# zakuro-ai/asr

Hardware: AMD Instinct MI355X
Metric: utterances/sec (10 s, 161-bin) DS2 5x1024 BiGRU CTC train step (higher is better)
Workload: dtype bf16

## Files before the change

### asr_amd/_lib.py

```python
from __future__ import annotations

import ctypes as C
import os
from typing import Optional

_HERE = os.path.dirname(os.path.abspath(__file__))
LIB_PATH = os.environ.get("DS2_LIB_PATH") or os.path.join(_HERE, "lib", "libds2hip.so")

_lib: Optional[C.CDLL] = None

vp, i32, i64, f32, f64, sz = C.c_void_p, C.c_int, C.c_longlong, C.c_float, C.c_double, C.c_size_t

SIGNATURES = {
    "ds2_version": (C.c_char_p, []),
    "ds2_last_error": (C.c_char_p, []),
    "ds2_device_info": (i32, [C.POINTER(i32), C.POINTER(i32), C.c_char_p, i32]),
    "ds2_debug_flags": (i32, [vp, i32]),
    "ds2_rnn_ctx_init": (i32, [vp, vp, vp, vp]),
    "ds2_memset_async": (i32, [vp, i32, sz, vp]),
    "ds2_ablation_build": (i32, []),
    "ds2_rnn_persistent_status": (i32, [vp, vp]),
    "ds2_rnn_persistent_counters": (i32, [vp, vp]),
    "ds2_rnn_poison_if_starved": (i32, [vp, vp, sz, vp]),
    "ds2_rnn_poison_seen": (i32, [vp]),
    "ds2_rnn_step_gate": (i32, [vp, vp, vp, vp]),
    "ds2_rnn_persistent_enable": (i32, [vp, i32, i32]),
    "ds2_rnn_last_path": (i32, [vp]),
    "ds2_rnn_bwd_ksplit_footprint": (i32, [i32, i32, C.POINTER(i32)]),
    "ds2_gemm_f32_workspace_bytes": (sz, [i32, i32, i32, i32]),
    "ds2_gemm_f32": (i32, [i32, i32, i32, i32, i32, vp, i32, i64, vp, i32, i64, vp, i32, i64, vp, i32, i32, i32, vp, sz, vp]),
    "ds2_gemm_bf16_workspace_bytes": (sz, [i32, i32, i32, i32]),
    "ds2_conv1_fwd_bf16_stat_blocks": (i32, [i32, i32, i32]),
    "ds2_conv1_fwd_bf16_stats": (i32, [vp, vp, vp, vp, vp, i32, i32, i32, vp, vp]),
    "ds2_conv2_fwd_bf16_stat_blocks": (i32, [i32, i32, i32]),
    "ds2_conv2_fwd_bf16_stats": (i32, [vp, vp, vp, vp, vp, i32, i32, i32, vp, vp]),
    "ds2_chanstats_from_partials_workspace_bytes": (sz, []),
    "ds2_chanstats_from_partials": (i32, [vp, i32, i32, f64, vp, vp, vp, vp, f32, vp, sz, vp]),
    "ds2_gemm_bf16_tn": (i32, [i32, i32, i32, vp, i32, i64, vp, i32, i64, vp, i32, i64, i32, i32, i32, vp, sz, vp]),
    "ds2_gemm_bf16_tn_group": (i32, [i32, vp, i32, vp]),
    "ds2_gemm_bf16_tn_splitk_group_workspace_bytes": (sz, [i32, vp, i32]),
    "ds2_gemm_bf16_tn_splitk_group": (i32, [i32, vp, i32, vp, sz, vp]),
    "ds2_gemm_bf16_tn_splitk_group_ep": (i32, [i32, vp, i32, i32, vp, vp, vp, vp, sz, vp]),
    "ds2_gemm_bf16_nt": (i32, [i32, i32, i32, vp, i32, i64, vp, i32, i64, vp, i32, i64, vp, i32, i32, i32, vp, sz, vp]),
    "ds2_cast_bf16": (i32, [vp, i32, vp, i32, i32, i32, vp]),
    "ds2_gemm_bf16_nt_obf16": (i32, [i32, i32, i32, vp, i32, vp, i32, vp, i32, vp, vp]),
    "ds2_cast_f32_from_bf16": (i32, [vp, vp, i64, vp]),
    "ds2_rnn_fwd_x": (i32, [vp, i32, vp, vp, vp, vp, vp, vp, vp, i32, i32, i32, vp, vp, vp, vp, sz, vp]),
    "ds2_split_bf16": (i32, [vp, i32, vp, i32, i32, i32, i32, vp]),
    "ds2_cast_transpose_bf16": (i32, [vp, i32, vp, i32, i32, i32, vp]),
    "ds2_cast_bf16_both_workspace_bytes": (sz, [i32, i32]),
    "ds2_cast_bf16_both": (i32, [vp, i32, vp, i32, vp, i32, i32, i32, vp, vp, sz, vp]),
    "ds2_transpose_bf16": (i32, [vp, i32, vp, i32, i32, i32, vp, vp, sz, vp]),
    "ds2_colreduce_workspace_bytes": (sz, [i32, i32]),
    "ds2_colstats_f32": (i32, [vp, i32, i32, i32, vp, vp, vp, vp, f32, vp, sz, vp]),
    "ds2_add_colstats_f32": (i32, [vp, i32, vp, i32, vp, i32, i32, i32, vp, vp, vp, vp, f32, vp, sz, vp]),
    "ds2_colsum_f32": (i32, [vp, i32, i32, i32, vp, vp, vp, sz, vp]),
    "ds2_bn1d_apply_f32": (i32, [vp, i32, vp, i32, i32, i32, vp, vp, vp, vp, f32, vp]),
    "ds2_bn1d_apply_bf16": (i32, [vp, i32, vp, i32, i32, i32, vp, vp, vp, vp, f32, vp]),
    "ds2_bn1d_bwd_f32": (i32, [vp, i32, vp, i32, vp, i32, i32, i32, vp, vp, vp, f32, vp, vp, vp, sz, vp]),
    "ds2_bn1d_bwd_xbf16": (i32, [vp, i32, vp, i32, vp, i32, i32, i32, vp, vp, vp, f32, vp, vp, vp, sz, vp]),
    "ds2_center_colstats": (i32, [vp, i32, vp, i32, vp, i32, vp, i32, i32, i32, vp, vp, vp, vp, vp, f32, vp, sz, vp]),
    "ds2_wih_fold_bf16": (i32, [vp, i32, vp, i32, i32, vp, vp, vp, vp, f32, vp, i32, vp, vp, vp, vp]),
    "ds2_scale_rank1_f32": (i32, [vp, i32, i32, i32, vp, vp, vp, vp]),
    "ds2_chanreduce_workspace_bytes": (sz, [i32]),
    "ds2_bn2d_stats_f32": (i32, [vp, i32, i32, i32, i32, vp, vp, vp, vp, f32, vp, sz, vp]),
# ... 150 lines not shown
```

### asr_amd/csrc/gemm_bf16.hip

```cpp
#include "common.h"
#include <type_traits>
#include <cstdint>
#include <stdlib.h>
#include <string.h>

namespace {

typedef __bf16 bf16x8 __attribute__((ext_vector_type(8)));
typedef __bf16 bf16x4 __attribute__((ext_vector_type(4)));
typedef float f32x2 __attribute__((ext_vector_type(2)));

constexpr int BM = 128, BN = 128, BK = 64;
constexpr int TN_MAX_PROBLEMS = 16;
constexpr int PITCH = 144;
constexpr int TILE_BYTES = BM * PITCH;

__device__ __attribute__((aligned(16))) float g_zero16[4] = {0.f, 0.f, 0.f, 0.f};
__device__ __attribute__((aligned(16))) float g_sink16[4];

struct BArgs {
  const __bf16* A; const __bf16* B; float* C; const float* bias;
  int M, N, K, lda, ldb, ldc;
  long long sA, sB, sC;
  int splitk, kchunk, accumulate;
// ... 986 lines not shown
    p.to_slab = nslab > 1;
    p.slab0 = term * splitk;
    p.nslab = (term == 0 && nslab > 1) ? nslab : 0;
    if (term == 0) {
      p.partial = (float*)((char*)workspace + off);
      if (nslab > 1) { off += (size_t)nslab * q.M * q.N * sizeof(float); elems += (long long)q.M * q.N / 4; any_slab = true; }
    } else {
      p.partial = g.p[i - term].partial;
    }
  }
  for (int i = nprob; i < TN_MAX_PROBLEMS; ++i) { g.p[i] = g.p[0]; g.p[i].nslab = 0; }
  g.nprob = nprob; g.splitk = splitk; g.nitems = items;
  g.ep_prob = ep_index; g.ep_scale = ep_scale; g.ep_rowv = ep_rowv; g.ep_shift = ep_shift;
  if (ep_index >= 0 && g.p[ep_index].nslab == 0) return 1;
  if (any_slab) DS2_REQUIRE(workspace && workspace_bytes >= off, "ds2_gemm_bf16_tn_splitk_group: workspace too small");
  DS2_ATTR_ONCE((gemm_bf16_tn_glds_kernel<true>), G_LDS);
  bool w4 = ds2_is_gfx950();
  for (int i = 0; i < nprob; ++i) {
    const ds2_tn_problem& q = probs[i];
    const int kc = g.p[i].kchunk, klast = q.K - (splitk - 1) * kc;
    w4 = w4 && (q.K % 64) == 0 && kc >= 128 && klast >= 128 && (long long)q.lda * 128 < (1ll << 31) && (long long)q.ldb * 128 < (1ll << 31);
  }
  if (w4) {
    DS2_ATTR_ONCE(gemm_bf16_tn_w4_kernel, W4_LDS);
    hipLaunchKernelGGL(gemm_bf16_tn_w4_kernel, dim3(items), dim3(256), W4_LDS, (hipStream_t)stream, g);
    DS2_LAUNCH_CHECK("gemm_bf16_tn_w4_kernel");
  } else {
    BArgs unused{};
    hipLaunchKernelGGL(gemm_bf16_tn_glds_kernel<true>, dim3(items), dim3(512), G_LDS, (hipStream_t)stream, unused, 0, 0, g);
    DS2_LAUNCH_CHECK("gemm_bf16_tn_glds_kernel<grouped>");
  }
  if (any_slab) {
    int blocks = (int)((elems + 255) / 256);
    if (blocks > 8192) blocks = 8192;
    hipLaunchKernelGGL(splitk_reduce_group_kernel, dim3(blocks), dim3(256), 0, (hipStream_t)stream, g, elems);
    DS2_LAUNCH_CHECK("splitk_reduce_group_kernel");
  }
  return 0;
}

extern "C" int ds2_gemm_bf16_tn_group(int nprob, const ds2_tn_problem* probs, int max_workgroups, void* stream) {
  DS2_REQUIRE(nprob >= 1 && nprob <= TNG_MAX_PROBLEMS && probs, "ds2_gemm_bf16_tn_group: 1..%d problems", TNG_MAX_PROBLEMS);
  TnGroup g;
  int tiles = 0;
  for (int i = 0; i < nprob; ++i) {
    const ds2_tn_problem& q = probs[i];
    DS2_REQUIRE(q.A && q.B && q.C && q.M >= 8 && q.N >= 8 && q.K > 0, "ds2_gemm_bf16_tn_group: problem %d: bad dims M=%d N=%d K=%d", i, q.M, q.N, q.K);
    DS2_REQUIRE((q.M % 8) == 0 && (q.N % 8) == 0 && (q.lda % 8) == 0 && (q.ldb % 8) == 0 && q.lda >= q.M && q.ldb >= q.N && q.ldc >= q.N,
                "ds2_gemm_bf16_tn_group: problem %d: M, N, lda, ldb must be multiples of 8 (M=%d N=%d lda=%d ldb=%d)", i, q.M, q.N, q.lda, q.ldb);
    DS2_REQUIRE(((uintptr_t)q.A % 16) == 0 && ((uintptr_t)q.B % 16) == 0, "ds2_gemm_bf16_tn_group: problem %d: operands must be 16-byte aligned", i);
    TnProb& p = g.p[i];
    p.A = (const __bf16*)q.A; p.B = (const __bf16*)q.B; p.C = q.C;
    p.M = q.M; p.N = q.N; p.K = q.K; p.lda = q.lda; p.ldb = q.ldb; p.ldc = q.ldc;
    p.ntx = ceil_div(q.N, 128);
    p.first_tile = tiles;
    tiles += p.ntx * ceil_div(q.M, 128);
  }
  for (int i = nprob; i < TNG_MAX_PROBLEMS; ++i) g.p[i] = g.p[0];
  g.nprob = nprob; g.ntiles = tiles;
  const int cus = ds2_cus_current() < 8 ? 8 : ds2_cus_current();
  int grid = max_workgroups > 0 ? (max_workgroups < cus ? max_workgroups : cus) : cus;
// ... 132 lines not shown
```

### asr_amd/csrc/gemm_tn_w4.h

```cpp
__global__ __launch_bounds__(256) void gemm_bf16_tn_w4_kernel(TnSGroup grp) {
  extern __shared__ __attribute__((aligned(1024))) char ldsg[];
  const __bf16* A;
  const __bf16* B;
  int pM, pN, plda, pldb, zs, orig, nt, kchunk, ntx, pK;
  float* Cfinal; float* Cslab; long long ldcf;
  bool partial;
  {
    const int item = tn_item_order(grp.nitems);
    A = grp.p[0].A; B = grp.p[0].B; Cfinal = grp.p[0].C; Cslab = grp.p[0].partial;
    pM = grp.p[0].M; pN = grp.p[0].N; pK = grp.p[0].K; plda = grp.p[0].lda; pldb = grp.p[0].ldb; ldcf = grp.p[0].ldc; ntx = grp.p[0].ntx;
    nt = grp.p[0].ntiles; kchunk = grp.p[0].kchunk;
    int first = 0, slab0 = grp.p[0].slab0, to_slab = grp.p[0].to_slab;
#pragma unroll
    for (int k = 1; k < TN_MAX_PROBLEMS; ++k)
      if (k < grp.nprob && item >= grp.p[k].first_item) {
        A = grp.p[k].A; B = grp.p[k].B; Cfinal = grp.p[k].C; Cslab = grp.p[k].partial;
        pM = grp.p[k].M; pN = grp.p[k].N; pK = grp.p[k].K; plda = grp.p[k].lda; pldb = grp.p[k].ldb; ldcf = grp.p[k].ldc; ntx = grp.p[k].ntx;
        nt = grp.p[k].ntiles; kchunk = grp.p[k].kchunk; first = grp.p[k].first_item; slab0 = grp.p[k].slab0; to_slab = grp.p[k].to_slab;
      }
    const int local = item - first;
    zs = local / nt; orig = local % nt;
    partial = to_slab != 0;
    Cslab += (long long)(slab0 + zs) * pM * pN;
  }
  const int m0 = (orig / ntx) * 256, n0 = (orig % ntx) * 256;
  const int kbeg = zs * kchunk;
  const int kend = min(pK, kbeg + kchunk);
  const int nkt = (kend - kbeg) >> 6;
  const int lane = threadIdx.x & 63;
  const int wave = __builtin_amdgcn_readfirstlane(threadIdx.x >> 6);
  const int wm = wave >> 1, wn = wave & 1;
  const unsigned lds0 = (unsigned)(uintptr_t)(lds_void*)ldsg;

  unsigned voffA[8], voffB[8];
#pragma unroll
  for (int i = 0; i < 8; ++i) {
    const int r = (wave + 4 * i) * 2 + (lane >> 5);
    const int gs = (lane & 31) ^ (((r & 3) << 2) | (((r >> 3) & 1) << 1));
    voffA[i] = (unsigned)(r * plda * 2 + min(m0 + gs * 8, pM - 8) * 2);
    voffB[i] = (unsigned)(r * pldb * 2 + min(n0 + gs * 8, pN - 8) * 2);
  }
  const char* sA = reinterpret_cast<const char*>(A + (long long)kbeg * plda);
  const char* sB = reinterpret_cast<const char*>(B + (long long)kbeg * pldb);
  const long long stepA = (long long)plda * 128, stepB = (long long)pldb * 128;
  const unsigned dstw = lds0 + wave * 1024;
  auto dma_a = [&](unsigned boff, int p) { w4_dma(voffA[p], sA, dstw + boff + p * 4096); };
  auto dma_b = [&](unsigned boff, int p) { w4_dma(voffB[p], sB, dstw + boff + 32768 + p * 4096); };

  const int p16 = lane & 15, q4 = p16 >> 2, g4 = lane >> 4;
  const unsigned rowpart = (unsigned)((g4 * 8 + q4) * 512);
  const unsigned xv = (unsigned)((q4 << 2) | ((g4 & 1) << 1));
  unsigned va[8], vb[8];
#pragma unroll
  for (int i = 0; i < 8; ++i) {
    const int ca = wm * 128 + i * 16 + 4 * (p16 & 3), cb = wn * 128 + i * 16 + 4 * (p16 & 3);
    va[i] = lds0 + rowpart + ((((ca >> 3) ^ xv) << 4) | (((ca >> 2) & 1) << 3));
    vb[i] = lds0 + 32768 + rowpart + ((((cb >> 3) ^ xv) << 4) | (((cb >> 2) & 1) << 3));
  }

  f32x4 acc[8][8];
  f32x4 fa[2][8], fb[2][8];
#define TW_BC(x) __builtin_bit_cast(bf16x8, x)
#define TW_SB() __builtin_amdgcn_sched_barrier(0)
#define TW_RD(dst, addr, off)                                                                                                         \
  do {                                                                                                                                \
    f32x2 lo_, hi_;                                                                                                                   \
    asm volatile("ds_read_b64_tr_b16 %0, %2 offset:%3\n\tds_read_b64_tr_b16 %1, %2 offset:%4"                                         \
                 : "=&v"(lo_), "=&v"(hi_)                                                                                             \
                 : "v"(addr), "n"(off), "n"((off) + 2048));                                                                           \
    dst = __builtin_shufflevector(lo_, hi_, 0, 1, 2, 3);                                                                              \
  } while (0)
#define TW_LGKM0(F)                                                                                                                   \
  asm volatile("s_waitcnt lgkmcnt(0)"                                                                                                 \
               : "+v"(F[0]), "+v"(F[1]), "+v"(F[2]), "+v"(F[3]), "+v"(F[4]), "+v"(F[5]), "+v"(F[6]), "+v"(F[7])                       \
               :                                                                                                                      \
               : "memory")
#define TW_KTILE(DMA, VMW, NEXT)                                                                                                      \
  do {                                                                                                                                \
    TW_SB();                                                                                                                          \
    _Pragma("unroll") for (int m_ = 0; m_ < 64; ++m_) {                                                                               \
      acc[m_ & 7][m_ >> 3] = __builtin_amdgcn_mfma_f32_16x16x32_bf16(TW_BC(fb[0][m_ >> 3]), TW_BC(fa[0][m_ & 7]), acc[m_ & 7][m_ >> 3], 0, 0, 0); \
// ... 13 lines not shown
    _Pragma("unroll") for (int m_ = 0; m_ < 64; ++m_) {                                                                               \
      acc[m_ & 7][m_ >> 3] = __builtin_amdgcn_mfma_f32_16x16x32_bf16(TW_BC(fb[1][m_ >> 3]), TW_BC(fa[1][m_ & 7]), acc[m_ & 7][m_ >> 3], 0, 0, 0); \
      TW_SB();                                                                                                                        \
      if ((DMA) && m_ < 10 && !(m_ & 1)) dma_b(boff, 3 + (m_ >> 1));                                                                  \
      if ((DMA) && m_ == 9) { sA += stepA; sB += stepB; }                                                                             \
      if ((NEXT) && m_ == 10) asm volatile(VMW ::: "memory");                                                                         \
      if ((NEXT) && m_ == 11) __builtin_amdgcn_s_barrier();                                                                           \
      if (m_ >= 13 && m_ <= 58 && (m_ - 13) % 3 == 0) {                                                                               \
        if ((m_ - 13) / 3 < 8) {                                                                                                      \
          va[((m_ - 13) / 3) & 7] ^= 65536u;                                                                                          \
          if (NEXT) TW_RD(fa[0][((m_ - 13) / 3) & 7], va[((m_ - 13) / 3) & 7], 0);                                                    \
        } else {                                                                                                                      \
          vb[((m_ - 13) / 3 - 8) & 7] ^= 65536u;                                                                                      \
          if (NEXT) TW_RD(fb[0][((m_ - 13) / 3 - 8) & 7], vb[((m_ - 13) / 3 - 8) & 7], 0);                                            \
        }                                                                                                                             \
      }                                                                                                                               \
      TW_SB();                                                                                                                        \
    }                                                                                                                                 \
    if (NEXT) { TW_LGKM0(fa[0]); TW_LGKM0(fb[0]); }                                                                                   \
    TW_SB();                                                                                                                          \
    boff ^= 65536u;                                                                                                                   \
  } while (0)

#pragma unroll
  for (int p = 0; p < 8; ++p) { dma_a(0u, p); dma_b(0u, p); }
  sA += stepA; sB += stepB;
#pragma unroll
  for (int p = 0; p < 8; ++p) { dma_a(65536u, p); dma_b(65536u, p); }
  sA += stepA; sB += stepB;
#pragma unroll
  for (int i = 0; i < 8; ++i)
#pragma unroll
    for (int j = 0; j < 8; ++j) acc[i][j] = f32x4{0.f, 0.f, 0.f, 0.f};
  asm volatile("s_waitcnt vmcnt(0)" ::: "memory");
  __builtin_amdgcn_s_barrier();
  TW_SB();
#pragma unroll
  for (int i = 0; i < 8; ++i) TW_RD(fa[0][i], va[i], 0);
#pragma unroll
  for (int j = 0; j < 8; ++j) TW_RD(fb[0][j], vb[j], 0);
  TW_LGKM0(fa[0]);
  TW_LGKM0(fb[0]);
  unsigned boff = 0u;
  int kt = 0;
  if (nkt > 2) {
    TW_KTILE(1, "", 1);
    kt = 1;
  }
  for (; kt < nkt - 2; ++kt) TW_KTILE(1, "s_waitcnt vmcnt(16)", 1);
  if (kt < nkt - 1) TW_KTILE(0, "s_waitcnt vmcnt(0)", 1);
  TW_KTILE(0, "", 0);

  {
    float* C = partial ? Cslab : Cfinal;
    const long long ldc = partial ? (long long)pN : ldcf;
    int el = lane;
    asm volatile("" : "+v"(el));
    const int frow = el & 15, fseg = el >> 4;
#pragma unroll
    for (int i = 0; i < 8; ++i) {
      const int row = m0 + wm * 128 + i * 16 + frow;
#pragma unroll
      for (int j = 0; j < 8; ++j) {
        const int col = n0 + wn * 128 + j * 16 + fseg * 4;
        if (row < pM && col < pN) *reinterpret_cast<f32x4*>(C + (long long)row * ldc + col) = acc[i][j];
      }
    }
  }
#undef TW_BC
#undef TW_SB
#undef TW_RD
#undef TW_LGKM0
#undef TW_KTILE
}
```

### asr_amd/engine.py

```python
from __future__ import annotations

from dataclasses import dataclass, field
from typing import Dict, List, Optional

import torch

from . import _lib, ops

Tensor = torch.Tensor
import os as _os
def _tune(name: str, default: str) -> str:
    return _os.environ.get(name, default) if _os.environ.get("DS2_EXPERIMENTAL") == "1" else default


OVERLAP_MODE = _tune("DS2_OVERLAP", "2")
OVERLAP_WGRAD = OVERLAP_MODE == "1"
WGRAD_TN = _tune("DS2_WGRAD_TN", "1") != "0"
CONV_STATS = _tune("DS2_CONV_STATS", "1") != "0"
FUSE_BN_BWD = _tune("DS2_FUSE_BN_BWD", "1") != "0"
WGRAD_SIDE = _tune("DS2_WGRAD_SIDE", "sk")
WGRAD_IDLE = _tune("DS2_WGRAD_IDLE", "1") != "0"
WGRAD_IDLE_MIN_CUS = int(_tune("DS2_WGRAD_IDLE_MIN_CUS", "64"))
F32_GEMM = _os.environ.get("DS2_F32_GEMM", "split")


F32_RNN = _os.environ.get("DS2_F32_RNN", "split")


F32_CONV = _os.environ.get("DS2_F32_CONV", "split")
F32_CONV_FWD = _tune("DS2_F32_CONV_FWD", "f32")
CONV2_WGRAD = _tune("DS2_CONV2_WGRAD", "nhwc")
GX_BF16 = _tune("DS2_GX_BF16", "0") != "0"
WS_PREARM = _tune("DS2_WS_PREARM", "1") != "0"
BN_FOLD = _tune("DS2_BN_FOLD", "1") != "0"
BN_FOLD_IDLE = _tune("DS2_BN_FOLD_IDLE", "1") != "0"


def _f32_split_ok(M: int, N: int, K: int, H: int = 8) -> bool:
    return F32_GEMM == "split" and M >= 512 and N >= 256 and K >= 256 and K % 8 == 0 and N % 8 == 0 and H % 8 == 0


_BWD_PERSISTENT = {}
_SIDE = {}
# ... 324 lines not shown
        rows = 2 * H if G == 3 else G * H
        ra, rb = (slice(B, M), slice(0, M - B)), (slice(0, M - B), slice(B, M))
        ops.gemm_bf16_tn_pair(dgx_bf[ra[0], 0:rows], dgx_bf[ra[1], G * H:G * H + rows], h_bf[rb[0], 0:H], h_bf[rb[1], H:2 * H], dwhh[:, :rows])
        if G == 3:
            ops.gemm_bf16_tn_pair(dhn_bf[ra[0], 0:H], dhn_bf[ra[1], H:2 * H], h_bf[rb[0], 0:H], h_bf[rb[1], H:2 * H], dwhh[:, 2 * H:])
        dwih = Gr[f"rnns.{l}.wih_cat"]
        I = dwih.shape[1]
        if I % 8 == 0:
            ops.gemm_bf16_tn(dgx_bf, xn[:, :I], out=dwih)
        else:
            dwih.copy_(ops.gemm_bf16_tn(dgx_bf, xn)[:, :I])
        fold_epilogue(l)
        done(f"rnns.{l}")

    def weight_gradients_group(l, dgx_bf, dhn_bf, h_bf, xn, on_side, start):
        dwhh, dwih = Gr[f"rnns.{l}.whh_cat"], Gr[f"rnns.{l}.wih_cat"]
        rows = 2 * H if G == 3 else G * H
        probs = [(dgx_bf, xn[:, :dwih.shape[1]], dwih),
                 (dgx_bf[B:M, 0:rows], h_bf[0:M - B, 0:H], dwhh[0, :rows]),
                 (dgx_bf[0:M - B, G * H:G * H + rows], h_bf[B:M, H:2 * H], dwhh[1, :rows])]
        if G == 3:
            probs += [(dhn_bf[B:M, 0:H], h_bf[0:M - B, 0:H], dwhh[0, 2 * H:]), (dhn_bf[0:M - B, H:2 * H], h_bf[B:M, H:2 * H], dwhh[1, 2 * H:])]
        f = fold_of.get(l)
        if WGRAD_SIDE == "sk" and f:
            def launch(pr):
                ops.gemm_bf16_tn_splitk_group(pr, epilogue=(0, f[0], Gr[f"rnns.{l}.bih_cat"].view(-1), f[1]))
        elif WGRAD_SIDE == "sk":
            launch = ops.gemm_bf16_tn_splitk_group
        else:
            def launch(pr):
                ops.gemm_bf16_tn_group(pr)
                fold_epilogue(l)
        if not on_side:
            launch(probs)
            done(f"rnns.{l}")
            return
        with torch.cuda.stream(side):
            side.wait_event(start)
            launch(probs)
            if not serial_buckets:
                done(f"rnns.{l}")
        if serial_buckets:
            main.wait_stream(side)
            done(f"rnns.{l}")
        for t in (dgx_bf, dhn_bf, h_bf, xn):
            if t is not None:
                t.record_stream(side)
        ctx.side_used = True

    shape_key = (ops.rnn_ctx_key(dev), G, H, B)

# ... 347 lines not shown
```

### asr_amd/ops.py

```python
from __future__ import annotations

import ctypes as C
import math
import threading
from typing import Optional, Tuple

import torch

from . import _lib

Tensor = torch.Tensor
BN_EPS = 1e-5
BN_MOMENTUM = 0.1


def _ptr(t: Optional[Tensor]):
    return None if t is None else t.data_ptr()


def _stream():
    return torch.cuda.current_stream().cuda_stream


def _chk_f32(*ts):
# ... 358 lines not shown
                break
            rounds = -(-tiles * s_ // 256)
            util = tiles * s_ / (rounds * 256.0)
            cost = 2.0 * mn * kmin / (1.1e15 * util) + (0.0 if s_ == 1 else (s_ + 1) * mn * 4 / 3e12)
            if best_cost is None or cost < best_cost * 0.97:
                best, best_cost = s_, cost
        splitk = best
    ap = C.cast(arr, C.c_void_p)
    wsb = lib.ds2_gemm_bf16_tn_splitk_group_workspace_bytes(len(problems), ap, splitk)
    ws = _ws(wsb, problems[0][0].device) if wsb else None
    if epilogue is not None:
        idx, scale, rowv, shift = epilogue
        _chk_f32(scale, rowv, shift)
        rc = lib.ds2_gemm_bf16_tn_splitk_group_ep(len(problems), ap, splitk, int(idx), scale.data_ptr(), rowv.data_ptr(), shift.data_ptr(), _ptr(ws), wsb, _stream())
        if rc == 0:
            return splitk
        if rc != 1:
            _lib.check(rc, "ds2_gemm_bf16_tn_splitk_group_ep")
        _lib.check(lib.ds2_gemm_bf16_tn_splitk_group(len(problems), ap, splitk, _ptr(ws), wsb, _stream()), "ds2_gemm_bf16_tn_splitk_group")
        scale_rank1_(problems[idx][2], scale, rowv, shift)
        return splitk
    _lib.check(lib.ds2_gemm_bf16_tn_splitk_group(len(problems), ap, splitk, _ptr(ws), wsb, _stream()), "ds2_gemm_bf16_tn_splitk_group")
    return splitk


def gemm_bf16_tn_group(problems, max_workgroups: int = 0):
    lib = _lib.load()
    arr = (_lib.TnProblem * len(problems))()
    for q, (A, B, out) in zip(arr, problems):
        assert A.dtype == torch.bfloat16 and B.dtype == torch.bfloat16 and out.dtype == torch.float32 and A.is_cuda and B.is_cuda and out.is_cuda
        assert A.dim() == 2 and B.dim() == 2 and out.dim() == 2 and A.stride(1) == 1 and B.stride(1) == 1 and out.stride(1) == 1
        K, M = A.shape
        assert B.size(0) == K and tuple(out.shape) == (M, B.size(1)), (A.shape, B.shape, out.shape)
        q.A, q.B, q.C = A.data_ptr(), B.data_ptr(), out.data_ptr()
        q.M, q.N, q.K, q.lda, q.ldb, q.ldc = M, B.size(1), K, _row_pitch(A), _row_pitch(B), _row_pitch(out)
    _lib.check(lib.ds2_gemm_bf16_tn_group(len(problems), C.cast(arr, C.c_void_p), int(max_workgroups), _stream()), "ds2_gemm_bf16_tn_group")


def colstats(X: Tensor, run_mean: Optional[Tensor] = None, run_var: Optional[Tensor] = None):
    _chk_f32(X, run_mean, run_var)
    lib = _lib.load()
    M, H = X.shape
    mean = torch.empty(H, dtype=torch.float32, device=X.device)
    var = torch.empty_like(mean)
    wsb = lib.ds2_colreduce_workspace_bytes(M, H)
    ws = _ws(wsb, X.device)
# ... 1191 lines not shown
```

### include/ds2hip.h

```cpp
#ifndef DS2HIP_H
#define DS2HIP_H

#include <stddef.h>
#include <stdint.h>

#ifdef __cplusplus
extern "C" {
#endif

const char* ds2_version(void);
const char* ds2_last_error(void);
int ds2_device_info(int* cu_count, int* wave_size, char* arch, int arch_len);
int ds2_ablation_build(void);

typedef struct ds2_rnn_ctx {
  int size;
  int persist_fwd, persist_bwd;
  int cooldown;
  int rearm_calls;
  int starved_total;
  int last_path;
  int last_bwd_kind;
  int debug_flags;
  int ws_prearmed;
// ... 9 lines not shown
size_t ds2_gemm_f32_workspace_bytes(int M, int N, int batch, int splitk);
int ds2_gemm_f32(int transA, int transB, int M, int N, int K, const float* A, int lda, long long strideA, const float* B, int ldb,
                 long long strideB, float* C, int ldc, long long strideC, const float* bias, int accumulate, int batch, int splitk,
                 void* workspace, size_t workspace_bytes, void* stream);

size_t ds2_gemm_bf16_workspace_bytes(int M, int N, int batch, int splitk);
int ds2_gemm_bf16_nt(int M, int N, int K, const void* A, int lda, long long strideA, const void* B, int ldb, long long strideB, float* C,
                     int ldc, long long strideC, const float* bias, int accumulate, int batch, int splitk, void* workspace,
                     size_t workspace_bytes, void* stream);
int ds2_gemm_bf16_nt_obf16(int M, int N, int K, const void* A, int lda, const void* B, int ldb, void* C, int ldc, const float* bias, void* stream);
int ds2_cast_f32_from_bf16(const void* src, float* dst, long long n, void* stream);
int ds2_gemm_bf16_tn(int M, int N, int K, const void* A, int lda, long long strideA, const void* B, int ldb, long long strideB, float* C,
                     int ldc, long long strideC, int accumulate, int batch, int splitk, void* workspace, size_t workspace_bytes,
                     void* stream);
typedef struct ds2_tn_problem {
  const void* A; const void* B; float* C;
  int M, N, K, lda, ldb, ldc;
} ds2_tn_problem;
int ds2_gemm_bf16_tn_group(int nprob, const ds2_tn_problem* problems, int max_workgroups, void* stream);
size_t ds2_gemm_bf16_tn_splitk_group_workspace_bytes(int nprob, const ds2_tn_problem* problems, int splitk);
int ds2_gemm_bf16_tn_splitk_group(int nprob, const ds2_tn_problem* problems, int splitk, void* workspace, size_t workspace_bytes, void* stream);
int ds2_gemm_bf16_tn_splitk_group_ep(int nprob, const ds2_tn_problem* probs, int splitk, int ep_index, const float* ep_scale, const float* ep_rowv,
                                     const float* ep_shift, void* workspace, size_t workspace_bytes, void* stream);
int ds2_cast_bf16(const float* src, int ld_src, void* dst, int ld_dst, int R, int Cc, void* stream);
int ds2_split_bf16(const float* src, int ld_src, void* dst, int ld_dst, int R, int Cc, int order, void* stream);
int ds2_cast_transpose_bf16(const float* src, int ld_src, void* dst, int ld_dst, int R, int Cc, void* stream);
size_t ds2_cast_bf16_both_workspace_bytes(int R, int Cc);
int ds2_cast_bf16_both(const float* src, int ld_src, void* dst_r, int ld_r, void* dst_t, int ld_t, int R, int Cc, float* colsum, void* ws,
                       size_t ws_bytes, void* stream);
int ds2_transpose_bf16(const void* src, int ld_src, void* dst_t, int ld_t, int R, int Cc, float* colsum, void* ws, size_t ws_bytes,
                       void* stream);

size_t ds2_colreduce_workspace_bytes(int M, int H);
int ds2_colstats_f32(const float* X, int ldx, int M, int H, float* mean, float* var, float* run_mean, float* run_var, float momentum,
                     void* ws, size_t ws_bytes, void* stream);
int ds2_add_colstats_f32(const float* Xa, int lda, const float* Xb, int ldb, float* Y, int ldy, int M, int H, float* mean, float* var,
                         float* run_mean, float* run_var, float momentum, void* ws, size_t ws_bytes, void* stream);
int ds2_colsum_f32(const float* X, int ldx, int M, int H, float* sum, float* sumsq, void* ws, size_t ws_bytes, void* stream);
int ds2_bn1d_apply_f32(const float* X, int ldx, float* Y, int ldy, int M, int H, const float* mean, const float* var,
                       const float* gamma, const float* beta, float eps, void* stream);
int ds2_bn1d_apply_bf16(const float* X, int ldx, void* Y, int ldy, int M, int H, const float* mean, const float* var, const float* gamma,
                        const float* beta, float eps, void* stream);
int ds2_bn1d_bwd_f32(const float* dY, int lddy, const float* X, int ldx, float* dX, int lddx, int M, int H, const float* mean,
                     const float* var, const float* gamma, float eps, float* dgamma, float* dbeta, void* ws, size_t ws_bytes,
                     void* stream);

// ... 244 lines not shown
```

Before: 2803.

## Add stream-K style run-partitioned grouped TN wgrad GEMM with cached host plans

Adds a persistent 'runs' variant of the w4 grouped TN GEMM. A host-side planner cuts the total K-tile work across all problems into near-equal contiguous runs, one per workgroup sized to the CU count. Each workgroup loops over its segments and writes partial tiles to slabs, which are reduced afterwards. Plans and device tables are cached per shape. The aim is to remove load imbalance and tail waves from fixed split-K for the RNN weight-gradient GEMMs, at the cost of extra slab traffic and a reduction pass. It is enabled by default for non-side-stream launches and falls back to split-K when the shapes are ineligible.

```diff
diff --git a/asr_amd/_lib.py b/asr_amd/_lib.py
--- a/asr_amd/_lib.py
+++ b/asr_amd/_lib.py
@@ -41,6 +41,9 @@
     "ds2_gemm_bf16_tn_splitk_group_workspace_bytes": (sz, [i32, vp, i32]),
     "ds2_gemm_bf16_tn_splitk_group": (i32, [i32, vp, i32, vp, sz, vp]),
     "ds2_gemm_bf16_tn_splitk_group_ep": (i32, [i32, vp, i32, i32, vp, vp, vp, vp, sz, vp]),
+    "ds2_gemm_bf16_tn_runs_group_workspace_bytes": (sz, [i32, vp, i32]),
+    "ds2_gemm_bf16_tn_runs_group": (i32, [i32, vp, i32, vp, sz, vp]),
+    "ds2_gemm_bf16_tn_runs_group_ep": (i32, [i32, vp, i32, i32, vp, vp, vp, vp, sz, vp]),
     "ds2_gemm_bf16_nt": (i32, [i32, i32, i32, vp, i32, i64, vp, i32, i64, vp, i32, i64, vp, i32, i32, i32, vp, sz, vp]),
     "ds2_cast_bf16": (i32, [vp, i32, vp, i32, i32, i32, vp]),
     "ds2_gemm_bf16_nt_obf16": (i32, [i32, i32, i32, vp, i32, vp, i32, vp, i32, vp, vp]),
diff --git a/asr_amd/csrc/gemm_bf16.hip b/asr_amd/csrc/gemm_bf16.hip
--- a/asr_amd/csrc/gemm_bf16.hip
+++ b/asr_amd/csrc/gemm_bf16.hip
@@ -1,4 +1,7 @@
 #include "common.h"
+#include "tn_runs_plan.h"
+#include <map>
+#include <mutex>
 #include <type_traits>
 #include <cstdint>
 #include <stdlib.h>
@@ -1032,8 +1035,9 @@
     w4 = w4 && (q.K % 64) == 0 && kc >= 128 && klast >= 128 && (long long)q.lda * 128 < (1ll << 31) && (long long)q.ldb * 128 < (1ll << 31);
   }
   if (w4) {
-    DS2_ATTR_ONCE(gemm_bf16_tn_w4_kernel, W4_LDS);
-    hipLaunchKernelGGL(gemm_bf16_tn_w4_kernel, dim3(items), dim3(256), W4_LDS, (hipStream_t)stream, g);
+    DS2_ATTR_ONCE((gemm_bf16_tn_w4_kernel<false>), W4_LDS);
+    hipLaunchKernelGGL((gemm_bf16_tn_w4_kernel<false>), dim3(items), dim3(256), W4_LDS, (hipStream_t)stream, g, (const TnRunsSeg*)nullptr,
+                       (const int*)nullptr);
     DS2_LAUNCH_CHECK("gemm_bf16_tn_w4_kernel");
   } else {
     BArgs unused{};
@@ -1047,6 +1051,126 @@
     DS2_LAUNCH_CHECK("splitk_reduce_group_kernel");
   }
   return 0;
+}
+
+namespace {
+struct TnRunsCached {
+  TnRunsPlan plan;
+  void* table = nullptr;
+  size_t seg_off = 0;
+};
+std::mutex g_tn_runs_mutex;
+std::map<std::vector<int>, TnRunsCached>& tn_runs_cache() { static std::map<std::vector<int>, TnRunsCached> c; return c; }
+
+bool tn_runs_eligible(int nprob, const ds2_tn_problem* probs) {
+  if (nprob < 1 || nprob > TN_MAX_PROBLEMS || !probs || !ds2_is_gfx950()) return false;
+  for (int i = 0; i < nprob; ++i) {
+    const ds2_tn_problem& q = probs[i];
+    if (q.K < 128 || (q.K % 64) != 0 || q.M < 8 || q.N < 8) return false;
+    if ((long long)q.lda * 128 >= (1ll << 31) || (long long)q.ldb * 128 >= (1ll << 31)) return false;
+    if (i > 0 && probs[i - 1].C == q.C) return false;
+  }
+  return true;
+}
+TnRunsCached* tn_runs_lookup(int nprob, const ds2_tn_problem* probs, int max_workgroups, bool upload, void* stream) {
+  int gmax = ds2_cus_current();
+  if (max_workgroups > 0 && max_workgroups < gmax) gmax = max_workgroups;
+  std::vector<int> key{ds2_dev_index(), gmax, nprob};
+  int Ms[TN_MAX_PROBLEMS], Ns[TN_MAX_PROBLEMS], Ks[TN_MAX_PROBLEMS];
+  for (int i = 0; i < nprob; ++i) {
+    Ms[i] = probs[i].M; Ns[i] = probs[i].N; Ks[i] = probs[i].K;
+    key.push_back(Ms[i]); key.push_back(Ns[i]); key.push_back(Ks[i]);
+  }
+  const int G = tn_runs_pick_groups(tn_runs_tiles(nprob, Ms, Ns), gmax);
+  std::lock_guard<std::mutex> lock(g_tn_runs_mutex);
+  auto& cache = tn_runs_cache();
+  auto it = cache.find(key);
+  if (it == cache.end()) {
+    if (cache.size() >= 256) return nullptr;
+    TnRunsCached c;
+    if (!tn_runs_plan(nprob, Ms, Ns, Ks, G, &c.plan)) return nullptr;
+    if (!c.plan.nphase && G != gmax && !tn_runs_plan(nprob, Ms, Ns, Ks, gmax, &c.plan)) return nullptr;
+    it = cache.emplace(key, std::move(c)).first;
+  }
+  TnRunsCached& c = it->second;
+  if (upload && !c.table) {
+    hipStreamCaptureStatus cap = hipStreamCaptureStatusNone;
+    if (hipStreamIsCapturing((hipStream_t)stream, &cap) != hipSuccess || cap != hipStreamCaptureStatusNone) return nullptr;
+    c.seg_off = ((size_t)(c.plan.G + 1) * sizeof(int) + 31) / 32 * 32;
+    const size_t bytes = c.seg_off + c.plan.segs.size() * sizeof(TnRunsSeg);
+    std::vector<char> host(bytes, 0);
+    memcpy(host.data(), c.plan.wg_first.data(), (size_t)(c.plan.G + 1) * sizeof(int));
+    if (!c.plan.segs.empty()) memcpy(host.data() + c.seg_off, c.plan.segs.data(), c.plan.segs.size() * sizeof(TnRunsSeg));
+    void* d = nullptr;
+    if (hipMalloc(&d, bytes) != hipSuccess) return nullptr;
+    if (hipMemcpy(d, host.data(), bytes, hipMemcpyHostToDevice) != hipSuccess) { (void)hipFree(d); return nullptr; }
+    c.table = d;
+  }
+  return &c;
+}
+
+int tn_runs_group_impl(int nprob, const ds2_tn_problem* probs, int max_workgroups, int ep_index, const float* ep_scale, const float* ep_rowv,
+                       const float* ep_shift, void* workspace, size_t workspace_bytes, void* stream) {
+  DS2_REQUIRE(nprob >= 1 && nprob <= TN_MAX_PROBLEMS && probs, "ds2_gemm_bf16_tn_runs_group: 1..%d problems", TN_MAX_PROBLEMS);
+  for (int i = 0; i < nprob; ++i) {
+    const ds2_tn_problem& q = probs[i];
+    DS2_REQUIRE(q.A && q.B && q.C && q.M >= 8 && q.N >= 8 && q.K > 0, "ds2_gemm_bf16_tn_runs_group: problem %d: bad dims M=%d N=%d K=%d", i, q.M, q.N, q.K);
+    DS2_REQUIRE((q.M % 8) == 0 && (q.N % 8) == 0 && (q.lda % 8) == 0 && (q.ldb % 8) == 0 && (q.ldc % 4) == 0 && ((uintptr_t)q.C % 16) == 0,
+                "ds2_gemm_bf16_tn_runs_group: problem %d: M, N, lda, ldb must be multiples of 8, ldc of 4, C 16-byte aligned", i);
+    DS2_REQUIRE(((uintptr_t)q.A % 16) == 0 && ((uintptr_t)q.B % 16) == 0, "ds2_gemm_bf16_tn_runs_group: problem %d: operands must be 16-byte aligned", i);
+  }
+  if (!tn_runs_eligible(nprob, probs)) return 1;
+  const TnRunsCached* c = tn_runs_lookup(nprob, probs, max_workgroups, true, stream);
+  if (!c) return 1;
+  TnSGroup g;
+  size_t off = 0;
+  long long elems = 0;
+  for (int i = 0; i < nprob; ++i) {
+    const ds2_tn_problem& q = probs[i];
+    TnSProb& p = g.p[i];
+    p.A = (const __bf16*)q.A; p.B = (const __bf16*)q.B; p.C = q.C;
+    p.M = q.M; p.N = q.N; p.K = q.K; p.lda = q.lda; p.ldb = q.ldb; p.ldc = q.ldc;
+    p.ntx = ceil_div(q.N, 256); p.ntiles = p.ntx * ceil_div(q.M, 256); p.kchunk = q.K; p.first_item = 0; p.slab0 = 0;
+    const bool slabs = c->plan.nslab[i] > 1 || i == ep_index;
+    p.to_slab = slabs; p.nslab = slabs ? c->plan.nslab[i] : 0;
+    p.partial = (float*)((char*)workspace + off);
+    if (slabs) { off += (size_t)p.nslab * q.M * q.N * sizeof(float); elems += (long long)q.M * q.N / 4; }
+  }
+  for (int i = nprob; i < TN_MAX_PROBLEMS; ++i) { g.p[i] = g.p[0]; g.p[i].nslab = 0; }
+  g.nprob = nprob; g.splitk = 1; g.nitems = 0;
+  g.ep_prob = ep_index; g.ep_scale = ep_scale; g.ep_rowv = ep_rowv; g.ep_shift = ep_shift;
+  if (off) DS2_REQUIRE(workspace && workspace_bytes >= off, "ds2_gemm_bf16_tn_runs_group: workspace too small");
+  DS2_ATTR_ONCE((gemm_bf16_tn_w4_kernel<true>), W4_LDS);
+  hipLaunchKernelGGL((gemm_bf16_tn_w4_kernel<true>), dim3(c->plan.G), dim3(256), W4_LDS, (hipStream_t)stream, g,
+                     (const TnRunsSeg*)((const char*)c->table + c->seg_off), (const int*)c->table);
+  DS2_LAUNCH_CHECK("gemm_bf16_tn_w4_kernel<runs>");
+  if (elems) {
+    int blocks = (int)((elems + 255) / 256);
+    if (blocks > 8192) blocks = 8192;
+    hipLaunchKernelGGL(splitk_reduce_group_kernel, dim3(blocks), dim3(256), 0, (hipStream_t)stream, g, elems);
+    DS2_LAUNCH_CHECK("splitk_reduce_group_kernel");
+  }
+  return 0;
+}
+}
+
+extern "C" size_t ds2_gemm_bf16_tn_runs_group_workspace_bytes(int nprob, const ds2_tn_problem* probs, int max_workgroups) {
+  if (!tn_runs_eligible(nprob, probs)) return 0;
+  const TnRunsCached* c = tn_runs_lookup(nprob, probs, max_workgroups, false, nullptr);
+  if (!c) return 0;
+  size_t n = 0;
+  for (int i = 0; i < nprob; ++i) n += (size_t)c->plan.nslab[i] * probs[i].M * probs[i].N * sizeof(float);
+  return n;
+}
+extern "C" int ds2_gemm_bf16_tn_runs_group(int nprob, const ds2_tn_problem* probs, int max_workgroups, void* workspace, size_t workspace_bytes,
+                                           void* stream) {
+  return tn_runs_group_impl(nprob, probs, max_workgroups, -1, nullptr, nullptr, nullptr, workspace, workspace_bytes, stream);
+}
+extern "C" int ds2_gemm_bf16_tn_runs_group_ep(int nprob, const ds2_tn_problem* probs, int max_workgroups, int ep_index, const float* ep_scale,
+                                              const float* ep_rowv, const float* ep_shift, void* workspace, size_t workspace_bytes, void* stream) {
+  DS2_REQUIRE(ep_index >= 0 && ep_index < nprob && ep_scale && ep_rowv && ep_shift && ((uintptr_t)ep_scale % 16) == 0 && ((uintptr_t)ep_shift % 16) == 0,
+              "ds2_gemm_bf16_tn_runs_group_ep: bad epilogue arguments");
+  return tn_runs_group_impl(nprob, probs, max_workgroups, ep_index, ep_scale, ep_rowv, ep_shift, workspace, workspace_bytes, stream);
 }
 
 extern "C" int ds2_gemm_bf16_tn_group(int nprob, const ds2_tn_problem* probs, int max_workgroups, void* stream) {
diff --git a/asr_amd/csrc/gemm_tn_w4.h b/asr_amd/csrc/gemm_tn_w4.h
--- a/asr_amd/csrc/gemm_tn_w4.h
+++ b/asr_amd/csrc/gemm_tn_w4.h
@@ -1,11 +1,52 @@
-__global__ __launch_bounds__(256) void gemm_bf16_tn_w4_kernel(TnSGroup grp) {
+template <bool RUNS>
+__global__ __launch_bounds__(256) void gemm_bf16_tn_w4_kernel(TnSGroup grp, const TnRunsSeg* __restrict__ segs, const int* __restrict__ wg_first) {
   extern __shared__ __attribute__((aligned(1024))) char ldsg[];
+  const int lane = threadIdx.x & 63;
+  const int wave = __builtin_amdgcn_readfirstlane(threadIdx.x >> 6);
+  const int wm = wave >> 1, wn = wave & 1;
+  const unsigned lds0 = (unsigned)(uintptr_t)(lds_void*)ldsg;
+  int seg = 0, seg_end = 1;
+  if constexpr (RUNS) {
+    seg = wg_first[blockIdx.x]; seg_end = wg_first[blockIdx.x + 1];
+    if (seg >= seg_end) return;
+  }
+
+  const int p16 = lane & 15, q4 = p16 >> 2, g4 = lane >> 4;
+  const unsigned rowpart = (unsigned)((g4 * 8 + q4) * 512);
+  const unsigned xv = (unsigned)((q4 << 2) | ((g4 & 1) << 1));
+  unsigned va[8], vb[8];
+#pragma unroll
+  for (int i = 0; i < 8; ++i) {
+    const int ca = wm * 128 + i * 16 + 4 * (p16 & 3), cb = wn * 128 + i * 16 + 4 * (p16 & 3);
+    va[i] = lds0 + rowpart + ((((ca >> 3) ^ xv) << 4) | (((ca >> 2) & 1) << 3));
+    vb[i] = lds0 + 32768 + rowpart + ((((cb >> 3) ^ xv) << 4) | (((cb >> 2) & 1) << 3));
+  }
+
+ for (;;) {
   const __bf16* A;
   const __bf16* B;
-  int pM, pN, plda, pldb, zs, orig, nt, kchunk, ntx, pK;
+  int pM, pN, plda, pldb, ntx, pK;
   float* Cfinal; float* Cslab; long long ldcf;
   bool partial;
-  {
+  int m0, n0, kbeg, nkt;
+  if constexpr (RUNS) {
+    const int4 d0 = *reinterpret_cast<const int4*>(segs + seg), d1 = *(reinterpret_cast<const int4*>(segs + seg) + 1);
+    const int prob = d0.x;
+    A = grp.p[0].A; B = grp.p[0].B; Cfinal = grp.p[0].C; Cslab = grp.p[0].partial;
+    pM = grp.p[0].M; pN = grp.p[0].N; pK = grp.p[0].K; plda = grp.p[0].lda; pldb = grp.p[0].ldb; ldcf = grp.p[0].ldc; ntx = grp.p[0].ntx;
+    int to_slab = grp.p[0].to_slab;
+#pragma unroll
+    for (int k = 1; k < TN_MAX_PROBLEMS; ++k)
+      if (k == prob) {
+        A = grp.p[k].A; B = grp.p[k].B; Cfinal = grp.p[k].C; Cslab = grp.p[k].partial;
+        pM = grp.p[k].M; pN = grp.p[k].N; pK = grp.p[k].K; plda = grp.p[k].lda; pldb = grp.p[k].ldb; ldcf = grp.p[k].ldc; ntx = grp.p[k].ntx;
+        to_slab = grp.p[k].to_slab;
+      }
+    m0 = d0.y; n0 = d0.z; kbeg = d0.w; nkt = d1.x;
+    partial = to_slab != 0;
+    Cslab += (long long)d1.y * pM * pN;
+  } else {
+    int zs, orig, nt, kchunk;
     const int item = tn_item_order(grp.nitems);
     A = grp.p[0].A; B = grp.p[0].B; Cfinal = grp.p[0].C; Cslab = grp.p[0].partial;
     pM = grp.p[0].M; pN = grp.p[0].N; pK = grp.p[0].K; plda = grp.p[0].lda; pldb = grp.p[0].ldb; ldcf = grp.p[0].ldc; ntx = grp.p[0].ntx;
@@ -22,15 +63,10 @@
     zs = local / nt; orig = local % nt;
     partial = to_slab != 0;
     Cslab += (long long)(slab0 + zs) * pM * pN;
-  }
-  const int m0 = (orig / ntx) * 256, n0 = (orig % ntx) * 256;
-  const int kbeg = zs * kchunk;
-  const int kend = min(pK, kbeg + kchunk);
-  const int nkt = (kend - kbeg) >> 6;
-  const int lane = threadIdx.x & 63;
-  const int wave = __builtin_amdgcn_readfirstlane(threadIdx.x >> 6);
-  const int wm = wave >> 1, wn = wave & 1;
-  const unsigned lds0 = (unsigned)(uintptr_t)(lds_void*)ldsg;
+    m0 = (orig / ntx) * 256; n0 = (orig % ntx) * 256;
+    kbeg = zs * kchunk;
+    nkt = (min(pK, kbeg + kchunk) - kbeg) >> 6;
+  }
 
   unsigned voffA[8], voffB[8];
 #pragma unroll
@@ -46,17 +82,6 @@
   const unsigned dstw = lds0 + wave * 1024;
   auto dma_a = [&](unsigned boff, int p) { w4_dma(voffA[p], sA, dstw + boff + p * 4096); };
   auto dma_b = [&](unsigned boff, int p) { w4_dma(voffB[p], sB, dstw + boff + 32768 + p * 4096); };
-
-  const int p16 = lane & 15, q4 = p16 >> 2, g4 = lane >> 4;
-  const unsigned rowpart = (unsigned)((g4 * 8 + q4) * 512);
-  const unsigned xv = (unsigned)((q4 << 2) | ((g4 & 1) << 1));
-  unsigned va[8], vb[8];
-#pragma unroll
-  for (int i = 0; i < 8; ++i) {
-    const int ca = wm * 128 + i * 16 + 4 * (p16 & 3), cb = wn * 128 + i * 16 + 4 * (p16 & 3);
-    va[i] = lds0 + rowpart + ((((ca >> 3) ^ xv) << 4) | (((ca >> 2) & 1) << 3));
-    vb[i] = lds0 + 32768 + rowpart + ((((cb >> 3) ^ xv) << 4) | (((cb >> 2) & 1) << 3));
-  }
 
   f32x4 acc[8][8];
   f32x4 fa[2][8], fb[2][8];
@@ -116,34 +141,39 @@
     boff ^= 65536u;                                                                                                                   \
   } while (0)
 
-#pragma unroll
-  for (int p = 0; p < 8; ++p) { dma_a(0u, p); dma_b(0u, p); }
-  sA += stepA; sB += stepB;
-#pragma unroll
-  for (int p = 0; p < 8; ++p) { dma_a(65536u, p); dma_b(65536u, p); }
-  sA += stepA; sB += stepB;
+  const bool work = !RUNS || nkt > 0;
+  if (work) {
+#pragma unroll
+    for (int p = 0; p < 8; ++p) { dma_a(0u, p); dma_b(0u, p); }
+    sA += stepA; sB += stepB;
+#pragma unroll
+    for (int p = 0; p < 8; ++p) { dma_a(65536u, p); dma_b(65536u, p); }
+    sA += stepA; sB += stepB;
+  }
 #pragma unroll
   for (int i = 0; i < 8; ++i)
 #pragma unroll
     for (int j = 0; j < 8; ++j) acc[i][j] = f32x4{0.f, 0.f, 0.f, 0.f};
-  asm volatile("s_waitcnt vmcnt(0)" ::: "memory");
-  __builtin_amdgcn_s_barrier();
-  TW_SB();
-#pragma unroll
-  for (int i = 0; i < 8; ++i) TW_RD(fa[0][i], va[i], 0);
-#pragma unroll
-  for (int j = 0; j < 8; ++j) TW_RD(fb[0][j], vb[j], 0);
-  TW_LGKM0(fa[0]);
-  TW_LGKM0(fb[0]);
-  unsigned boff = 0u;
-  int kt = 0;
-  if (nkt > 2) {
-    TW_KTILE(1, "", 1);
-    kt = 1;
-  }
-  for (; kt < nkt - 2; ++kt) TW_KTILE(1, "s_waitcnt vmcnt(16)", 1);
-  if (kt < nkt - 1) TW_KTILE(0, "s_waitcnt vmcnt(0)", 1);
-  TW_KTILE(0, "", 0);
+  if (work) {
+    asm volatile("s_waitcnt vmcnt(0)" ::: "memory");
+    __builtin_amdgcn_s_barrier();
+    TW_SB();
+#pragma unroll
+    for (int i = 0; i < 8; ++i) TW_RD(fa[0][i], va[i], 0);
+#pragma unroll
+    for (int j = 0; j < 8; ++j) TW_RD(fb[0][j], vb[j], 0);
+    TW_LGKM0(fa[0]);
+    TW_LGKM0(fb[0]);
+    unsigned boff = 0u;
+    int kt = 0;
+    if (nkt > 2) {
+      TW_KTILE(1, "", 1);
+      kt = 1;
+    }
+    for (; kt < nkt - 2; ++kt) TW_KTILE(1, "s_waitcnt vmcnt(16)", 1);
+    if (kt < nkt - 1) TW_KTILE(0, "s_waitcnt vmcnt(0)", 1);
+    TW_KTILE(0, "", 0);
+  }
 
   {
     float* C = partial ? Cslab : Cfinal;
@@ -161,6 +191,13 @@
       }
     }
   }
+  if constexpr (!RUNS) break;
+  if (++seg >= seg_end) break;
+  if (nkt & 1) {
+#pragma unroll
+    for (int i = 0; i < 8; ++i) { va[i] ^= 65536u; vb[i] ^= 65536u; }
+  }
+ }
 #undef TW_BC
 #undef TW_SB
 #undef TW_RD
diff --git a/asr_amd/csrc/tn_runs_plan.h b/asr_amd/csrc/tn_runs_plan.h
--- /dev/null
+++ b/asr_amd/csrc/tn_runs_plan.h
@@ -0,0 +1,121 @@
+#pragma once
+#include <cstdint>
+#include <vector>
+
+struct TnRunsSeg {
+  int prob, m0, n0, kbeg;
+  int nkt, slab, tile, pad;
+};
+
+struct TnRunsPlan {
+  int G = 0, ntiles = 0, nphase = 0, even_k = 0;
+  long long len_spread = 0;
+  std::vector<long long> cut;
+  std::vector<int> run_of_wg;
+  std::vector<int> wg_first;
+  std::vector<TnRunsSeg> segs;
+  std::vector<int> nslab;
+  std::vector<int> tile_prob, tile_nkt;
+};
+
+inline int tn_runs_gcd(int a, int b) { while (b) { const int t = a % b; a = b; b = t; } return a; }
+
+inline int tn_runs_tiles(int nprob, const int* M, const int* N) {
+  int T = 0;
+  for (int p = 0; p < nprob; ++p) T += ((M[p] + 255) / 256) * ((N[p] + 255) / 256);
+  return T;
+}
+inline int tn_runs_pick_groups(int ntiles, int gmax) {
+  for (int G = gmax - gmax % 8; G >= 8 && 4 * G >= 3 * gmax; G -= 8)
+    if (8 % (G / tn_runs_gcd(ntiles, G)) == 0) return G;
+  return gmax;
+}
+
+inline bool tn_runs_plan(int nprob, const int* M, const int* N, const int* K, int G, TnRunsPlan* out) {
+  if (nprob < 1 || G < 1) return false;
+  struct Tile { int prob, m0, n0, nkt; };
+  std::vector<Tile> base;
+  int kmin = 0, kmax = 0;
+  for (int p = 0; p < nprob; ++p) {
+    if (M[p] < 1 || N[p] < 1 || K[p] < 128 || (K[p] % 64) != 0) return false;
+    const int nkt = K[p] / 64, ntx = (N[p] + 255) / 256, nty = (M[p] + 255) / 256;
+    kmin = (p == 0 || nkt < kmin) ? nkt : kmin;
+    kmax = (p == 0 || nkt > kmax) ? nkt : kmax;
+    for (int c0 = 0; c0 < ntx; c0 += 8)
+      for (int r = 0; r < nty; ++r)
+        for (int c = c0; c < ntx && c < c0 + 8; ++c) base.push_back(Tile{p, r * 256, c * 256, nkt});
+  }
+  const int T = (int)base.size();
+  TnRunsPlan& pl = *out;
+  pl = TnRunsPlan();
+  pl.G = G; pl.ntiles = T;
+  pl.even_k = (kmax - kmin) <= kmax / 64;
+  const int g = tn_runs_gcd(T, G), P = G / g, Q = T / g, bs = G / 8;
+  pl.nphase = (pl.even_k && (G % 8) == 0 && (8 % P) == 0) ? P : 0;
+  pl.len_spread = pl.even_k ? ((long long)T * (kmax - kmin) + G - 1) / G + 6 : 5;
+
+  std::vector<Tile> line(base);
+  if (pl.nphase && Q > 1)
+    for (int grp = 0; grp < T / (Q * bs); ++grp)
+      for (int c = 0; c < Q; ++c)
+        for (int j = 0; j < bs; ++j) line[grp * Q * bs + Q * j + c] = base[grp * Q * bs + c * bs + j];
+  std::vector<long long> start(T + 1, 0);
+  for (int t = 0; t < T; ++t) start[t + 1] = start[t] + line[t].nkt;
+  const long long L = start[T];
+  pl.tile_prob.resize(T); pl.tile_nkt.resize(T);
+  for (int t = 0; t < T; ++t) { pl.tile_prob[t] = line[t].prob; pl.tile_nkt[t] = line[t].nkt; }
+
+  pl.cut.assign(G + 1, 0);
+  pl.cut[G] = L;
+  int t = 0;
+  for (int r = 1; r < G; ++r) {
+    long long off;
+    if (pl.even_k) {
+      const long long num = (long long)r * T;
+      t = (int)(num / G);
+      off = ((num % G) * line[t].nkt + G / 2) / G;
+    } else {
+      const long long c = (long long)r * L / G;
+      while (start[t + 1] <= c) ++t;
+      off = c - start[t];
+    }
+    const long long prev = pl.cut[r - 1];
+    const long long lo = prev > start[t] ? prev - start[t] : 0;
+    if (off - lo < 2) off = lo;
+    else if (line[t].nkt - off < 2) off = line[t].nkt;
+    pl.cut[r] = start[t] + off;
+  }
+
+  std::vector<int> used(T, 0), last_run(T, -1);
+  std::vector<std::vector<TnRunsSeg>> of_run(G);
+  t = 0;
+  for (int r = 0; r < G; ++r) {
+    long long a = pl.cut[r];
+    const long long b = pl.cut[r + 1];
+    while (a < b) {
+      while (start[t + 1] <= a) ++t;
+      const long long e = b < start[t + 1] ? b : start[t + 1];
+      of_run[r].push_back(TnRunsSeg{line[t].prob, line[t].m0, line[t].n0, (int)(a - start[t]) * 64, (int)(e - a), used[t]++, t, 0});
+      last_run[t] = r;
+      a = e;
+    }
+  }
+  pl.nslab.assign(nprob, 0);
+  for (int i = 0; i < T; ++i) pl.nslab[line[i].prob] = used[i] > pl.nslab[line[i].prob] ? used[i] : pl.nslab[line[i].prob];
+  for (int i = 0; i < T; ++i)
+    for (int s = used[i]; s < pl.nslab[line[i].prob]; ++s)
+      of_run[last_run[i]].push_back(TnRunsSeg{line[i].prob, line[i].m0, line[i].n0, 0, 0, s, i, 0});
+
+  pl.run_of_wg.resize(G);
+  for (int w = 0; w < G; ++w) {
+    const int x = w & 7;
+    pl.run_of_wg[w] = pl.nphase ? P * ((x / P) * bs + (w >> 3)) + (x % P) : w;
+  }
+  pl.wg_first.assign(G + 1, 0);
+  for (int w = 0; w < G; ++w) {
+    const std::vector<TnRunsSeg>& v = of_run[pl.run_of_wg[w]];
+    pl.segs.insert(pl.segs.end(), v.begin(), v.end());
+    pl.wg_first[w + 1] = (int)pl.segs.size();
+  }
+  return true;
+}
diff --git a/asr_amd/engine.py b/asr_amd/engine.py
--- a/asr_amd/engine.py
+++ b/asr_amd/engine.py
@@ -19,6 +19,7 @@
 CONV_STATS = _tune("DS2_CONV_STATS", "1") != "0"
 FUSE_BN_BWD = _tune("DS2_FUSE_BN_BWD", "1") != "0"
 WGRAD_SIDE = _tune("DS2_WGRAD_SIDE", "sk")
+WGRAD_RUNS = _tune("DS2_WGRAD_RUNS", "1") != "0"
 WGRAD_IDLE = _tune("DS2_WGRAD_IDLE", "1") != "0"
 WGRAD_IDLE_MIN_CUS = int(_tune("DS2_WGRAD_IDLE_MIN_CUS", "64"))
 F32_GEMM = _os.environ.get("DS2_F32_GEMM", "split")
@@ -389,11 +390,11 @@
         if G == 3:
             probs += [(dhn_bf[B:M, 0:H], h_bf[0:M - B, 0:H], dwhh[0, 2 * H:]), (dhn_bf[0:M - B, H:2 * H], h_bf[B:M, H:2 * H], dwhh[1, 2 * H:])]
         f = fold_of.get(l)
-        if WGRAD_SIDE == "sk" and f:
+        if WGRAD_SIDE == "sk":
             def launch(pr):
-                ops.gemm_bf16_tn_splitk_group(pr, epilogue=(0, f[0], Gr[f"rnns.{l}.bih_cat"].view(-1), f[1]))
-        elif WGRAD_SIDE == "sk":
-            launch = ops.gemm_bf16_tn_splitk_group
+                ep = (0, f[0], Gr[f"rnns.{l}.bih_cat"].view(-1), f[1]) if f else None
+                if not (WGRAD_RUNS and not on_side and ops.gemm_bf16_tn_runs_group(pr, epilogue=ep)):
+                    ops.gemm_bf16_tn_splitk_group(pr, epilogue=ep)
         else:
             def launch(pr):
                 ops.gemm_bf16_tn_group(pr)
diff --git a/asr_amd/ops.py b/asr_amd/ops.py
--- a/asr_amd/ops.py
+++ b/asr_amd/ops.py
@@ -404,6 +404,27 @@
         return splitk
     _lib.check(lib.ds2_gemm_bf16_tn_splitk_group(len(problems), ap, splitk, _ptr(ws), wsb, _stream()), "ds2_gemm_bf16_tn_splitk_group")
     return splitk
+
+
+def gemm_bf16_tn_runs_group(problems, max_workgroups: int = 0, epilogue=None) -> bool:
+    lib = _lib.load()
+    arr = _tn_problem_array(problems)
+    ap = C.cast(arr, C.c_void_p)
+    wsb = lib.ds2_gemm_bf16_tn_runs_group_workspace_bytes(len(problems), ap, int(max_workgroups))
+    if not wsb:
+        return False
+    ws = _ws(wsb, problems[0][0].device)
+    if epilogue is not None:
+        idx, scale, rowv, shift = epilogue
+        _chk_f32(scale, rowv, shift)
+        rc = lib.ds2_gemm_bf16_tn_runs_group_ep(len(problems), ap, int(max_workgroups), int(idx), scale.data_ptr(), rowv.data_ptr(), shift.data_ptr(),
+                                                _ptr(ws), wsb, _stream())
+    else:
+        rc = lib.ds2_gemm_bf16_tn_runs_group(len(problems), ap, int(max_workgroups), _ptr(ws), wsb, _stream())
+    if rc == 1:
+        return False
+    _lib.check(rc, "ds2_gemm_bf16_tn_runs_group")
+    return True
 
 
 def gemm_bf16_tn_group(problems, max_workgroups: int = 0):
diff --git a/include/ds2hip.h b/include/ds2hip.h
--- a/include/ds2hip.h
+++ b/include/ds2hip.h
@@ -55,6 +55,10 @@
 int ds2_gemm_bf16_tn_splitk_group(int nprob, const ds2_tn_problem* problems, int splitk, void* workspace, size_t workspace_bytes, void* stream);
 int ds2_gemm_bf16_tn_splitk_group_ep(int nprob, const ds2_tn_problem* probs, int splitk, int ep_index, const float* ep_scale, const float* ep_rowv,
                                      const float* ep_shift, void* workspace, size_t workspace_bytes, void* stream);
+size_t ds2_gemm_bf16_tn_runs_group_workspace_bytes(int nprob, const ds2_tn_problem* problems, int max_workgroups);
+int ds2_gemm_bf16_tn_runs_group(int nprob, const ds2_tn_problem* problems, int max_workgroups, void* workspace, size_t workspace_bytes, void* stream);
+int ds2_gemm_bf16_tn_runs_group_ep(int nprob, const ds2_tn_problem* probs, int max_workgroups, int ep_index, const float* ep_scale,
+                                   const float* ep_rowv, const float* ep_shift, void* workspace, size_t workspace_bytes, void* stream);
 int ds2_cast_bf16(const float* src, int ld_src, void* dst, int ld_dst, int R, int Cc, void* stream);
 int ds2_split_bf16(const float* src, int ld_src, void* dst, int ld_dst, int R, int Cc, int order, void* stream);
 int ds2_cast_transpose_bf16(const float* src, int ld_src, void* dst, int ld_dst, int R, int Cc, void* stream);
```

After: 2814 (median of 5 runs). About the same (+0.4%).
